# HongMJ1315/Path_Tracing

Hardware: AMD Instinct MI355X
Metric: Msamples/s (paths/s) at 1024^2 x 256spp (higher is better)
Workload: dtype f32; 1 GPU; configs[2]: unidirectional PT + NEE, Cornell-style box + tessellated sphere, 99024 triangles behind a BVH, 1024x1024, 256 spp, depth 4, 1 cone light; parallelism=image tiles 32x32 round-robin over 1 rank(s), RCCL gather to rank 0, seed=1

## Files before the change

### path_tracing_amd/csrc/hpt_host.h

```cpp
#pragma once
#include "../../include/hpt.h"
#include "hpt_scene.h"
#include "pt_kernels.h"
#include "bdpt_kernels.h"
#include "ppm_kernels.h"

#include <hip/hip_runtime.h>
#include <algorithm>
#include <cstring>
#include <string>
#include <vector>

namespace hpt {

int fail(int code, const std::string &msg);

inline int fail_hip(const std::string &what, hipError_t e){
    return fail(e == hipErrorOutOfMemory ? HPT_ERR_NOMEM : HPT_ERR_DEVICE, what + ": " + hipGetErrorString(e));
}

#define HIP_TRY(expr) do { hipError_t e_ = (expr); if(e_ != hipSuccess) return hpt::fail_hip(#expr, e_); } while(0)

template <typename T>
class DevBuf {
// ... 49 lines not shown
        hpt::DevBuf<hpt::DevMaterial> mats; hpt::DevBuf<hpt::DevLight> lights;
        hpt::DevBuf<float4> tri_frames;
        int stack_levels = hpt::kStackDepth;
        std::vector<unsigned char> h_lights, h_spheres, h_tris;
        int nl = 0, ns = 0, nt = 0;
        std::vector<int32_t> g_kind, g_index, g_group;
    } geo;

    struct PassBuffers {
        hpt::DevBuf<float4> org_eta, dir_flags, thr, col; hpt::DevBuf<uint2> rng, hit;
        hpt::DevBuf<float4> org_max, dir, contrib;
        hpt::PathBuf pb{}; hpt::ShadowBuf sb{};
        hpt::DevBuf<uint32_t> queue[2];
        hpt::DevBuf<uint32_t> squeue;
        hpt::DevBuf<uint32_t> lqueue[2];
        hpt::DevBuf<uint32_t> deep_stack;
        hpt::DevBuf<uint32_t> counters;
        uint32_t *h_count = nullptr;
        size_t cap_paths() const { return org_eta.capacity(); }
    };
    struct Workspace {
        PassBuffers pass[hpt::kMaxPipes];
        hipStream_t px_stream[hpt::kMaxPipes] = {}; int px_priority[hpt::kMaxPipes] = {};
        hipEvent_t px_fork = nullptr, px_done[hpt::kMaxPipes] = {};
        const uint32_t *last_counters = nullptr;
        int last_counter_stride = 0;
        int last_budget = 0;
        hpt::DevBuf<float4> accum;
        hpt::DevBuf<hpt::WorkCounters> wc;
        hpt::DevBuf<float> local_own, image_own;
// ... 93 lines not shown
```

### path_tracing_amd/csrc/pt_kernels.h

```cpp
#pragma once
#include <hip/hip_runtime.h>
#include <cstdint>
#include "hpt_scene.h"

namespace hpt {

struct SceneDev {
    const float4 *nodes;
    const uint4 *qnodes;
    const uint4 *wnodes;
    int wide_depth;
    float qorigin[3], qscale[3];
    const float4 *tris;
    const float4 *tri_frames;
    const DevRound *rounds;
    const DevMaterial *mats;
    const DevLight *lights;
    int num_rounds, num_spheres, num_lights, num_tris, num_mats, num_nodes;
};

struct PathBuf {
    float4 *org_eta;
    float4 *dir_flags;
    float4 *thr;
// ... 43 lines not shown
constexpr int kTraceBudget = HPT_TRACE_BUDGET;
constexpr int kTopLevels = HPT_TOP_LEVELS;
constexpr int kTopNodes = 1 << kTopLevels;

void launch_generate(hipStream_t s, const Tiling &tl, const CameraDev &cam, PathBuf pb,
                     uint32_t *qcount, int samples_this_pass, uint32_t first_sample, uint64_t seed,
                     WorkCounters *wc);
void launch_extend(hipStream_t s, const SceneDev &sc, PathBuf pb, const uint32_t *queue, const uint32_t *qcount,
                   uint32_t max_items, int flags, WorkCounters *wc);
void launch_shade(hipStream_t s, const SceneDev &sc, PathBuf pb, const uint32_t *queue, const uint32_t *qcount,
                  uint32_t max_items, uint32_t *next_queue, uint32_t *next_count, ShadowBuf sb, uint32_t *squeue,
                  uint32_t *scount, int max_depth, int max_delta, int roulette, WorkCounters *wc, const PrimaryGen *primary = nullptr,
                  uint32_t max_groups = 0);
void launch_connect(hipStream_t s, const SceneDev &sc, PathBuf pb, ShadowBuf sb, const uint32_t *squeue,
                    const uint32_t *scount, uint32_t max_items, int flags, WorkCounters *wc);
struct TraceSplit { uint32_t *equeue, *ecount, *squeue, *scount; int budget; };
void launch_trace(hipStream_t s, const SceneDev &sc, PathBuf pb, ShadowBuf sb, const uint32_t *equeue,
                  const uint32_t *ecount, uint32_t max_extend, const uint32_t *squeue, const uint32_t *scount,
                  uint32_t max_shadow, int stack_levels, bool count, WorkCounters *wc,
                  const TraceSplit *split = nullptr, const PrimaryGen *primary = nullptr, uint32_t max_groups = 0);
void launch_trace_resume(hipStream_t s, const SceneDev &sc, PathBuf pb, ShadowBuf sb, bool extend, bool shadow,
                         uint32_t max_items, WorkCounters *wc, const TraceSplit &split, const PrimaryGen *primary,
                         uint32_t max_groups, uint32_t *deep_stack);
inline bool resume_walk_fits(const SceneDev &sc){ return 3 * sc.wide_depth + 2 <= kResumeLdsLevels + kDeepLevels; }
size_t resume_deep_stack_words();
void launch_tri_frames(hipStream_t s, const float4 *tris, int num_tris, float4 *frames);
void launch_resolve(hipStream_t s, const Tiling &tl, PathBuf pb, float4 *accum, int samples_this_pass);
void launch_finalize(hipStream_t s, const Tiling &tl, const float4 *accum, float *d_local, float scale);
void launch_untile(hipStream_t s, const Tiling &tl, const float *d_gathered, float *d_image);

void launch_tonemap(hipStream_t s, const float *d_linear, void *d_bytes, unsigned long long num_values, int bgr, const float *d_thresholds);

void launch_probe_functions(hipStream_t s, const float *d_in, int n, float *d_out);
void launch_probe_closest(hipStream_t s, const SceneDev &sc, const float *org, const float *dir, int n, int flags,
                          float *t_out, int32_t *prim_out);
void launch_probe_visibility(hipStream_t s, const SceneDev &sc, const float *p1, const float *p2, int n, int flags,
                             int32_t *vis_out);

// ... 2 lines not shown
```

### path_tracing_amd/csrc/pt_kernels.hip

```cpp
#include "pt_kernels.h"
#include "pt_device_math.h"

namespace hpt {

namespace {

HPT_DEV uint32_t f2u(float f){ return __float_as_uint(f); }
HPT_DEV float u2f(uint32_t u){ return __uint_as_float(u); }
HPT_DEV f3 xyz(float4 v){ return mk3(v.x, v.y, v.z); }

HPT_DEV uint32_t bit_select(uint32_t m, uint32_t a, uint32_t b){ uint32_t r; asm("v_bfi_b32 %0, %1, %2, %3" : "=v"(r) : "v"(m), "v"(a), "v"(b)); return r; }
HPT_DEV float lo16f(uint32_t w){ float r; asm("v_cvt_f32_u32_sdwa %0, %1 dst_sel:DWORD dst_unused:UNUSED_PAD src0_sel:WORD_0" : "=v"(r) : "v"(w)); return r; }
HPT_DEV float hi16f(uint32_t w){ float r; asm("v_cvt_f32_u32_sdwa %0, %1 dst_sel:DWORD dst_unused:UNUSED_PAD src0_sel:WORD_1" : "=v"(r) : "v"(w)); return r; }

HPT_DEV uint32_t lds_push(bool want, uint32_t *lds_counter){
    unsigned long long mask = __ballot(want);
    if(mask == 0ull) return 0u;
    uint32_t lo = (uint32_t) mask, hi = (uint32_t) (mask >> 32);
    uint32_t prefix = __builtin_amdgcn_mbcnt_hi(hi, __builtin_amdgcn_mbcnt_lo(lo, 0u));
    uint32_t base = 0u;
    int leader = __ffsll((long long) mask) - 1;
    if((int) (threadIdx.x & 63u) == leader) base = atomicAdd(lds_counter, (uint32_t) __popcll(mask));
    base = (uint32_t) __shfl((int) base, leader, 64);
    return base + prefix;
// ... 215 lines not shown
        ++rays;
        if(COUNT) tally.wave_steps += wave_max_u32(tally.steps - s0);
    }
    if(COUNT) flush_tally(tally, rays, wc, false);
}

template <bool BRUTE, bool COUNT>
__global__ __launch_bounds__(kBlock)
void k_connect(SceneDev sc, PathBuf pb, ShadowBuf sb, const uint32_t *squeue, const uint32_t *scount, WorkCounters *wc){
    __shared__ uint32_t s_stack[kStackDepth * kBlock];
    uint32_t count = *scount;
    uint32_t *stk = s_stack + threadIdx.x;
    Tally tally; tally.boxes = 0; tally.tris = 0; tally.steps = 0; tally.wave_steps = 0;
    uint32_t rays = 0;
    for(uint32_t i = blockIdx.x * kBlock + threadIdx.x; i < count; i += gridDim.x * kBlock){
        uint32_t path = squeue[i];
        float4 a = sb.org_max[path], b = sb.dir[path];
        uint32_t s0 = tally.steps;
        bool vis = segment_visible<BRUTE, COUNT>(sc, xyz(a), xyz(b), a.w, stk, tally);
        ++rays;
        if(COUNT) tally.wave_steps += wave_max_u32(tally.steps - s0);
        if(vis){
            float4 c = sb.contrib[path];
            float4 col = pb.col[path];
            col.x = col.x + c.x; col.y = col.y + c.y; col.z = col.z + c.z;
            pb.col[path] = col;
        }
    }
    if(COUNT) flush_tally(tally, rays, wc, true);
}

#ifndef HPT_LDS_MATS
#define HPT_LDS_MATS 128
#endif
#ifndef HPT_LDS_LIGHTS
#define HPT_LDS_LIGHTS 32
#endif
#ifndef HPT_SHADE_CHUNK
// ... 13 lines not shown
#ifdef HPT_SHADE_PROFILE
#define HPT_SECTION(set, idx) do { if(wc && HPT_SHADE_PROFILE == (set)){ unsigned long long m_ = __ballot(true); \
    if((int) (threadIdx.x & 63u) == __ffsll((long long) m_) - 1){ atomicAdd(&wc->bd_pairs + 2 * (idx), 1ull); atomicAdd(&wc->bd_pairs + 2 * (idx) + 1, (unsigned long long) __popcll(m_)); } } } while(0)
#else
#define HPT_SECTION(set, idx) do {} while(0)
#endif

template <bool PRIMARY, bool STRIDED>
__global__ __launch_bounds__(kBlock) HPT_SHADE_ATTR
void k_shade(SceneDev sc, PathBuf pb, const uint32_t *queue, const uint32_t *qcount,
             uint32_t *next_queue, uint32_t *next_count, ShadowBuf sb, uint32_t *squeue, uint32_t *scount,
             int max_depth, int max_delta, int roulette, WorkCounters *wc, PrimaryGen pg){
    __shared__ DevMaterial s_mats[kLdsMats];
    __shared__ DevLight s_lights[kLdsLights];
    __shared__ uint32_t s_next[kShadeChunk];
    __shared__ uint32_t s_shadow[kShadeChunk];
    __shared__ uint32_t s_cnt[4];
    __shared__ uint32_t s_stage[kBlock / 64][kNeeWords][64];
    uint32_t (*stage)[64] = s_stage[threadIdx.x >> 6];
    uint32_t staged = 0u;
    const uint32_t lane = threadIdx.x & 63u;
    auto flush_nee = [&](uint32_t n){
        bool want = false; uint32_t spath = 0u;
        if(lane < n){
            HPT_SECTION(2, 3);
            f3 wo_l = mk3(u2f(stage[0][lane]), u2f(stage[1][lane]), u2f(stage[2][lane]));
            f3 wi_l = mk3(u2f(stage[3][lane]), u2f(stage[4][lane]), u2f(stage[5][lane]));
            ShadePre pre; pre.lam_o = u2f(stage[6][lane]);
            const uint32_t mat_i = stage[7][lane], light_i = stage[19][lane];
            f3 thr = mk3(u2f(stage[8][lane]), u2f(stage[9][lane]), u2f(stage[10][lane]));
            const float pdf_light_dir = u2f(stage[11][lane]);
            f3 p1 = mk3(u2f(stage[12][lane]), u2f(stage[13][lane]), u2f(stage[14][lane]));
            f3 p2 = mk3(u2f(stage[15][lane]), u2f(stage[16][lane]), u2f(stage[17][lane]));
            spath = stage[18][lane];
            const DevMaterial dm = (sc.num_mats <= kLdsMats ? s_mats : sc.mats)[mat_i];
            const DevLight &L = (sc.num_lights <= kLdsLights ? s_lights : sc.lights)[light_i & 0x7FFFFFFFu];
            Mat m; m.base = mk3(dm.base[0], dm.base[1], dm.base[2]); m.roughness = dm.roughness; m.metallic = dm.metallic; m.eta = dm.eta;
            pre.diffuse = mk3(dm.diffuse[0], dm.diffuse[1], dm.diffuse[2]);
// ... 4 lines not shown
            f3 contrib;
            if(light_i >> 31) contrib = thr * brdf * illum * mk3(1.0f, 1.0f, 1.0f) * cos_surface * (float) sc.num_lights;
            else {
                float p_l = pdf_light_dir * pdf_light_dir;
                float p_b = pdf_bsdf * pdf_bsdf;
                float mis_w = p_l / fmaxf(p_l + p_b, 1e-8f);
                contrib = thr * brdf * illum * mk3(1.0f, 1.0f, 1.0f) * cos_surface / pdf_light_dir * mis_w;
            }
            if(is_valid_color(contrib)){
                HPT_SECTION(5, 3);
                want = true;
                f3 c = clamp_radiance(contrib, 15.0f);
                f3 diff = p2 - p1;
                float dist = length3(diff);
                f3 dir = diff / dist;
                sb.org_max[spath] = make_float4(p1.x, p1.y, p1.z, dist - 1e-3f);
                sb.dir[spath] = make_float4(dir.x, dir.y, dir.z, 0.0f);
                sb.contrib[spath] = make_float4(c.x, c.y, c.z, 0.0f);
            }
        }
        uint32_t spos = lds_push(want, &s_cnt[1]);
        if(want) s_shadow[spos] = spath;
    };
#ifdef HPT_SHADE_PROFILE
    g_hpt_probe = wc ? &wc->bd_pairs : nullptr;
#endif
    if(threadIdx.x < 4) s_cnt[threadIdx.x] = 0u;
    const bool mats_in_lds = sc.num_mats <= kLdsMats;
    const bool lights_in_lds = sc.num_lights <= kLdsLights;
    if(mats_in_lds){
        const uint32_t *src = (const uint32_t *) sc.mats; uint32_t *dst = (uint32_t *) s_mats;
        for(int w = threadIdx.x; w < sc.num_mats * (int) (sizeof(DevMaterial) / 4); w += kBlock) dst[w] = src[w];
    }
    if(lights_in_lds){
        const uint32_t *src = (const uint32_t *) sc.lights; uint32_t *dst = (uint32_t *) s_lights;
        for(int w = threadIdx.x; w < sc.num_lights * (int) (sizeof(DevLight) / 4); w += kBlock) dst[w] = src[w];
    }
// ... 2 lines not shown
    const DevLight *lights = lights_in_lds ? s_lights : sc.lights;

    uint32_t count = *qcount;
    uint32_t chunk = (count + kShadeTargetGroups - 1) / kShadeTargetGroups;
    chunk = (chunk + kBlock - 1) / kBlock * kBlock;
    chunk = chunk < (uint32_t) kBlock ? (uint32_t) kBlock : (chunk > (uint32_t) kShadeChunk ? (uint32_t) kShadeChunk : chunk);
    uint32_t iters = 0;
    for(uint32_t cb = blockIdx.x; (unsigned long long) cb * chunk < count; cb += gridDim.x){
    if(STRIDED && cb != blockIdx.x){
        __syncthreads();
        if(threadIdx.x < 4) s_cnt[threadIdx.x] = 0u;
        __syncthreads();
    }
    uint32_t begin = cb * chunk;
    uint32_t end = begin + chunk < count ? begin + chunk : count;
    for(uint32_t base = begin; base < end; base += kBlock){
        uint32_t i = base + threadIdx.x;
        bool alive = false, nee = false;
        uint32_t path = 0;
        f3 n_wo = mk3(0, 0, 0), n_wi = mk3(0, 0, 0), n_thr = mk3(0, 0, 0), s_p1 = mk3(0, 0, 0), s_p2 = mk3(0, 0, 0);
        float n_lam = 0.0f, n_pdf_light = 0.0f; uint32_t n_mat = 0u, n_light = 0u;
        if(i < count){
            path = queue ? queue[i] : i;
            ++iters;
            HPT_SECTION(1, 0);
            uint2 h = pb.hit[path];
            uint32_t prim = h.y;
            f3 p_eye = mk3(0, 0, 0), p_dir = mk3(0, 0, 1), first_col = mk3(0, 0, 0); uint64_t p_rs = 0ull;
            if(PRIMARY && !primary_ray(pg, path, p_eye, p_dir, p_rs)) prim = kHitMiss;
            if(prim != kHitMiss){
// ... 200 lines not shown
                }
                staged += k;
            }
        }
        uint32_t qpos = lds_push(alive, &s_cnt[0]);
        if(alive) s_next[qpos] = path;
    }
    if(staged != 0u){ flush_nee(staged); staged = 0u; }
    __syncthreads();
    if(threadIdx.x == 0){
        s_cnt[2] = s_cnt[0] ? atomicAdd(next_count, s_cnt[0]) : 0u;
        s_cnt[3] = s_cnt[1] ? atomicAdd(scount, s_cnt[1]) : 0u;
    }
    __syncthreads();
    for(uint32_t k = threadIdx.x; k < s_cnt[0]; k += kBlock) next_queue[s_cnt[2] + k] = s_next[k];
    for(uint32_t k = threadIdx.x; k < s_cnt[1]; k += kBlock) squeue[s_cnt[3] + k] = s_shadow[k];
    if(!STRIDED) break;
    }
    if(wc){
        unsigned long long v = iters;
        for(int off = 32; off > 0; off >>= 1) v += __shfl_down(v, off, 64);
        if((threadIdx.x & 63u) == 0u && v) atomicAdd(&wc->path_iters, v);
    }
}

__global__ __launch_bounds__(kBlock)
void k_resolve(Tiling tl, PathBuf pb, float4 *accum, int samples){
    uint32_t p = blockIdx.x * kBlock + threadIdx.x;
    if(p >= (uint32_t) tl.n_local) return;
    float4 a = accum[p];
    f3 sum = mk3(a.x, a.y, a.z);
// ... 84 lines not shown
#if HPT_TRACE_WAVES > 0
#define HPT_TRACE_ATTR __attribute__((amdgpu_waves_per_eu(HPT_TRACE_WAVES, 8)))
#else
#define HPT_TRACE_ATTR
#endif
constexpr int kTraceChunk = 2048;
constexpr uint32_t kDoneCode = 0xFFFFFFFEu;
constexpr int kRefillMin = 56;
constexpr int kNodeMin = 4;
constexpr uint32_t kTraceShortQueue = 1u << 20;

template <bool ANY, bool COUNT, bool RESUME, bool TOP, bool PRIMARY>
HPT_DEV void trace_chunk(const SceneDev &sc, PathBuf pb, ShadowBuf sb, const uint32_t *queue,
                         uint32_t end, uint32_t *stk, uint32_t *s_next, int refill_min, int node_min, WorkCounters *wc,
                         uint32_t budget, uint32_t *s_long, uint32_t *s_nlong, const uint4 *top, const PrimaryGen &pg,
                         uint32_t *deep, uint32_t deep_stride){
    bool active = false, exhausted = false;
    uint32_t path = 0u, cur = 0u, steps = 0u;
    int sp = 0;
    f3 ro = mk3(0, 0, 0), rd = mk3(0, 0, 1);
    float ix = 0, iy = 0, iz = 0, ox = 0, oy = 0, oz = 0;
    uint32_t mx = 0u, my = 0u, mz = 0u;
    float tmax = 0.0f, limit = 0.0f, best_t = 1e20f;
    uint32_t best_prim = kHitMiss, best_ord = 0xFFFFFFFFu;
    unsigned long long n_lane_steps = 0, n_wave_steps = 0, n_boxes = 0, n_tris = 0, n_rays = 0, n_leaf_lane = 0, n_leaf_wave = 0;
    const uint32_t lane = threadIdx.x & 63u;
    const uint32_t step_limit = budget != 0u ? budget : 0xFFFFFFFFu;
    for(;;){
        if(!RESUME && budget != 0u){
            bool defer = active && steps >= budget;
            unsigned long long dm = __ballot(defer);
            if(dm != 0ull){
                uint32_t dn = (uint32_t) __popcll(dm);
                uint32_t dprefix = __builtin_amdgcn_mbcnt_hi((uint32_t) (dm >> 32), __builtin_amdgcn_mbcnt_lo((uint32_t) dm, 0u));
                int dleader = __ffsll((long long) dm) - 1;
                uint32_t dbase = 0u;
                if((int) lane == dleader) dbase = atomicAdd(s_nlong, dn);
                dbase = (uint32_t) __shfl((int) dbase, dleader, 64);
                if(defer){
                    s_long[dbase + dprefix] = path;
                    if(!ANY) pb.hit[path] = make_uint2(f2u(best_t), best_prim);
                    active = false;
                }
            }
        }
        unsigned long long idle = __ballot(!active);
        if(idle != 0ull && !exhausted && (idle == ~0ull || __popcll(idle) >= refill_min)){
            uint32_t n = (uint32_t) __popcll(idle);
            uint32_t prefix = __builtin_amdgcn_mbcnt_hi((uint32_t) (idle >> 32), __builtin_amdgcn_mbcnt_lo((uint32_t) idle, 0u));
            int leader = __ffsll((long long) idle) - 1;
            uint32_t base = 0u;
            if((int) lane == leader) base = atomicAdd(s_next, n);
            base = (uint32_t) __shfl((int) base, leader, 64);
            exhausted = base + n >= end;
            if(!active){
                uint32_t i = base + prefix;
                if(i < end){
                    path = queue ? queue[i] : i;
                    bool start = true;
                    if(ANY){
                        float4 a = sb.org_max[path], b = sb.dir[path];
                        ro = xyz(a); rd = xyz(b); tmax = a.w;
                        if(COUNT && !RESUME) n_rays += 1;
                        for(int r = 0; r < (RESUME ? 0 : sc.num_spheres); ++r){
                            DevRound rr = sc.rounds[r];
                            float t;
                            if(hit_sphere(ro, rd, mk3(rr.c[0], rr.c[1], rr.c[2]), rr.r, tmax, t) && t > 1e-3f && (rr.flags & 1u)) start = false;
                        }
                        limit = tmax;
                    } else {
                        bool outside;
                        if(PRIMARY){
                            uint64_t rs_unused;
                            outside = !primary_ray(pg, path, ro, rd, rs_unused);
                            if(outside && !RESUME) pb.hit[path] = make_uint2(f2u(1e20f), kHitMiss);
                        } else {
                            float4 o = pb.org_eta[path], d = pb.dir_flags[path];
                            ro = xyz(o); rd = xyz(d);
                            outside = (f2u(d.w) & 2u) != 0u;
                        }
                        if(outside) start = false;
                        else if(RESUME){
                            uint2 h = pb.hit[path];
                            best_t = u2f(h.x); best_prim = h.y; best_ord = 0xFFFFFFFFu;
                            if(best_prim != kHitMiss)
                                best_ord = (best_prim & kHitRoundFlag) ? (best_prim & ~kHitRoundFlag) : f2u(sc.tris[(size_t) best_prim * 3].w);
                            limit = best_t;
                        } else {
                            if(COUNT) n_rays += 1;
                            best_t = 1e20f; best_prim = kHitMiss; best_ord = 0xFFFFFFFFu;
                            for(int r = 0; r < sc.num_rounds; ++r){
                                DevRound rr = sc.rounds[r];
                                float t;
                                if(hit_sphere(ro, rd, mk3(rr.c[0], rr.c[1], rr.c[2]), rr.r, 1e20f, t) && t < best_t){
                                    best_t = t; best_prim = kHitRoundFlag | (uint32_t) r; best_ord = (uint32_t) r;
                                }
                            }
                            limit = best_t;
                        }
                    }
                    if(start){
                        float dx = fabsf(rd.x) > 1e-20f ? rd.x : copysignf(1e-20f, rd.x);
                        float dy = fabsf(rd.y) > 1e-20f ? rd.y : copysignf(1e-20f, rd.y);
// ... 115 lines not shown
                            }
                        }
                    }
                }
                if(ANY && blocked) finished = true;
                else if(sp > 0){
                    --sp;
                    cur = (RESUME && sp >= kResumeLdsLevels) ? deep[(size_t) (sp - kResumeLdsLevels) * deep_stride] : stk[sp * kBlock];
                }
                else finished = true;
            }
            if(finished){
                active = false;
                if(!ANY) pb.hit[path] = make_uint2(f2u(best_t), best_prim);
                else if(!blocked){
                    float4 c = sb.contrib[path];
                    float4 col = pb.col[path];
                    col.x = col.x + c.x; col.y = col.y + c.y; col.z = col.z + c.z;
                    pb.col[path] = col;
                }
            }
        }
    }
    if(COUNT){
        for(int off = 32; off > 0; off >>= 1){
            n_boxes += __shfl_down(n_boxes, off, 64); n_tris += __shfl_down(n_tris, off, 64);
            n_rays += __shfl_down(n_rays, off, 64); n_lane_steps += __shfl_down(n_lane_steps, off, 64);
            n_wave_steps += __shfl_down(n_wave_steps, off, 64); n_leaf_lane += __shfl_down(n_leaf_lane, off, 64);
            n_leaf_wave += __shfl_down(n_leaf_wave, off, 64);
        }
        if(lane == 0u){
            if(n_boxes) atomicAdd(ANY ? &wc->boxes_shadow : &wc->boxes_closest, n_boxes);
            if(n_tris) atomicAdd(ANY ? &wc->tris_shadow : &wc->tris_closest, n_tris);
            if(n_rays) atomicAdd(ANY ? &wc->shadow_rays : &wc->closest_rays, n_rays);
            if(n_lane_steps) atomicAdd(ANY ? &wc->lane_steps_shadow : &wc->lane_steps_closest, n_lane_steps);
            if(n_wave_steps) atomicAdd(ANY ? &wc->wave_steps_shadow : &wc->wave_steps_closest, n_wave_steps);
            if(n_leaf_lane) atomicAdd(ANY ? &wc->leaf_lane_shadow : &wc->leaf_lane_closest, n_leaf_lane);
            if(n_leaf_wave) atomicAdd(ANY ? &wc->leaf_wave_shadow : &wc->leaf_wave_closest, n_leaf_wave);
        }
    }
}

struct LongQueues { uint32_t *equeue, *ecount, *squeue, *scount; uint32_t budget; };

template <bool COUNT, bool RESUME, bool TOP, bool PRIMARY>
__global__ __launch_bounds__(kBlock) HPT_TRACE_ATTR
void k_trace(SceneDev sc, PathBuf pb, ShadowBuf sb, const uint32_t *equeue, const uint32_t *ecount_ptr,
             const uint32_t *squeue, const uint32_t *scount_ptr, uint32_t chunk_rays, int refill_min, int node_min,
             int stack_words, LongQueues lq, WorkCounters *wc, PrimaryGen pg, uint32_t *deep){
    extern __shared__ uint32_t s_dyn_stack[];
    __shared__ uint32_t s_next, s_nlong, s_gbase;
    __shared__ uint4 s_top[TOP ? kTopNodes * 2 : 1];
    uint32_t *s_long = s_dyn_stack + stack_words;
    if(TOP){
        const uint32_t words = (uint32_t) (sc.num_nodes < kTopNodes ? sc.num_nodes : kTopNodes) * 2u;
        for(uint32_t i = threadIdx.x; i < words; i += kBlock) s_top[i] = sc.qnodes[i];
    }
    uint32_t ecount = ecount_ptr ? *ecount_ptr : 0u, scount = scount_ptr ? *scount_ptr : 0u;
    uint32_t ce = ecount >= kTraceShortQueue ? chunk_rays : (uint32_t) kBlock;
    uint32_t cs = scount >= kTraceShortQueue ? chunk_rays : (uint32_t) kBlock;
    uint32_t ne = (ecount + ce - 1) / ce, ns = (scount + cs - 1) / cs;
    for(uint32_t bid = blockIdx.x; bid < ne + ns; bid += gridDim.x){
        bool shadow = bid >= ne;
        uint32_t chunk = shadow ? bid - ne : bid;
        uint32_t csize = shadow ? cs : ce;
        uint32_t begin = chunk * csize;
        uint32_t total = shadow ? scount : ecount;
        uint32_t end = begin + csize < total ? begin + csize : total;
        if(threadIdx.x == 0){ s_next = begin; s_nlong = 0u; }
        __syncthreads();
        uint32_t *deep_lane = RESUME ? deep + (size_t) blockIdx.x * kBlock + threadIdx.x : nullptr;
        const uint32_t deep_stride = gridDim.x * kBlock;
        if(shadow) trace_chunk<true, COUNT, RESUME, TOP, false>(sc, pb, sb, squeue, end, s_dyn_stack + threadIdx.x, &s_next, refill_min, node_min, wc,
                                                                lq.budget, s_long, &s_nlong, s_top, pg, deep_lane, deep_stride);
        else trace_chunk<false, COUNT, RESUME, TOP, PRIMARY>(sc, pb, sb, equeue, end, s_dyn_stack + threadIdx.x, &s_next, refill_min, node_min, wc,
                                                             lq.budget, s_long, &s_nlong, s_top, pg, deep_lane, deep_stride);
        __syncthreads();
        if(!RESUME && lq.budget != 0u){
            uint32_t n = s_nlong;
            if(n != 0u){
                if(threadIdx.x == 0) s_gbase = atomicAdd(shadow ? lq.scount : lq.ecount, n);
                __syncthreads();
                uint32_t *dst = (shadow ? lq.squeue : lq.equeue) + s_gbase;
                for(uint32_t i = threadIdx.x; i < n; i += kBlock) dst[i] = s_long[i];
            }
        }
        __syncthreads();
    }
}

template <bool BRUTE>
__global__ __launch_bounds__(kBlock)
void k_probe_closest(SceneDev sc, const float *org, const float *dir, int n, float *t_out, int32_t *prim_out){
    __shared__ uint32_t s_stack[kStackDepth * kBlock];
    int i = blockIdx.x * kBlock + threadIdx.x;
    if(i >= n) return;
    Tally tally; tally.boxes = 0; tally.tris = 0; tally.steps = 0; tally.wave_steps = 0;
    float t; uint32_t prim;
    closest_hit<BRUTE, false>(sc, mk3(org[3 * i], org[3 * i + 1], org[3 * i + 2]), mk3(dir[3 * i], dir[3 * i + 1], dir[3 * i + 2]),
// ... 121 lines not shown
    auto groups = [&](uint32_t items){
        uint32_t a = (items + chunk - 1) / chunk;
        uint32_t shortest = items < kTraceShortQueue ? items : kTraceShortQueue;
        uint32_t b = (shortest + kBlock - 1) / kBlock;
        return a > b ? a : b;
    };
    uint32_t g = (ecount ? groups(max_extend) : 0u) + (scount ? groups(max_shadow) : 0u);
    if(g == 0u) return;
    if(max_groups != 0u && g > max_groups) g = max_groups;
    if(stack_levels < 1) stack_levels = 1;
    if(stack_levels > kStackDepth) stack_levels = kStackDepth;
    int stack_words = (stack_levels + 1) * kBlock;
    LongQueues lq{};
    if(split && split->budget > 0 && !count){
        lq.equeue = split->equeue; lq.ecount = split->ecount; lq.squeue = split->squeue; lq.scount = split->scount;
        lq.budget = (uint32_t) split->budget;
        if(stack_levels > split->budget) stack_words = (split->budget + 1) * kBlock;
    }
    size_t lds = (size_t) stack_words * sizeof(uint32_t) + (lq.budget ? (size_t) chunk * sizeof(uint32_t) : 0);
    const bool top = lq.budget != 0u && lq.budget <= (uint32_t) kTopLevels;
    PrimaryGen none{};
    const PrimaryGen &pg = primary ? *primary : none;
#define HPT_LAUNCH_TRACE(C, T, P) hipLaunchKernelGGL((k_trace<C, false, T, P>), dim3(g), dim3(kBlock), lds, s, sc, pb, sb, equeue, ecount, squeue, \
                                                     scount, chunk, kRefillMin, kNodeMin, stack_words, lq, wc, pg, (uint32_t *) nullptr)
    if(count) HPT_LAUNCH_TRACE(true, false, false);
    else if(top && primary) HPT_LAUNCH_TRACE(false, true, true);
    else if(top) HPT_LAUNCH_TRACE(false, true, false);
    else if(primary) HPT_LAUNCH_TRACE(false, false, true);
    else HPT_LAUNCH_TRACE(false, false, false);
#undef HPT_LAUNCH_TRACE
}

void launch_trace_resume(hipStream_t s, const SceneDev &sc, PathBuf pb, ShadowBuf sb, bool extend, bool shadow,
                         uint32_t max_items, WorkCounters *wc, const TraceSplit &split, const PrimaryGen *primary,
                         uint32_t max_groups, uint32_t *deep_stack){
    if(!extend && !shadow) return;
    const int stack_words = (kResumeLdsLevels + 1) * kBlock;
    const size_t lds = (size_t) stack_words * sizeof(uint32_t);
    uint32_t per = (max_items + kBlock - 1) / kBlock;
    uint64_t g = (uint64_t) per * ((extend ? 1u : 0u) + (shadow ? 1u : 0u));
    uint32_t g2 = g < kResumeMaxGroups ? (uint32_t) (g < 1u ? 1u : g) : kResumeMaxGroups;
    if(max_groups != 0u && g2 > max_groups) g2 = max_groups;
    LongQueues none{};
    PrimaryGen no_primary{};
    const uint32_t *eq = extend ? split.equeue : nullptr, *ec = extend ? split.ecount : nullptr;
    const uint32_t *sq = shadow ? split.squeue : nullptr, *scn = shadow ? split.scount : nullptr;
#define HPT_LAUNCH_RESUME(P, PG) hipLaunchKernelGGL((k_trace<false, true, false, P>), dim3(g2), dim3(kBlock), lds, s, sc, pb, sb, eq, ec, sq, scn, \
                                                    kLongChunk, kWideRefillMin, kWideNodeMin, stack_words, none, wc, PG, deep_stack)
    if(primary && extend) HPT_LAUNCH_RESUME(true, *primary);
    else HPT_LAUNCH_RESUME(false, no_primary);
#undef HPT_LAUNCH_RESUME
}

size_t resume_deep_stack_words(){ return (size_t) kDeepLevels * kResumeMaxGroups * kBlock; }

void launch_tri_frames(hipStream_t s, const float4 *tris, int num_tris, float4 *frames){
    if(num_tris <= 0) return;
    hipLaunchKernelGGL(k_tri_frames, dim3((num_tris + kBlock - 1) / kBlock), dim3(kBlock), 0, s, tris, num_tris, frames);
}

void launch_resolve(hipStream_t s, const Tiling &tl, PathBuf pb, float4 *accum, int samples_this_pass){
    uint32_t g = ((uint32_t) tl.n_local + kBlock - 1) / kBlock;
    hipLaunchKernelGGL(k_resolve, dim3(g), dim3(kBlock), 0, s, tl, pb, accum, samples_this_pass);
}

void launch_finalize(hipStream_t s, const Tiling &tl, const float4 *accum, float *d_local, float divisor){
// ... 37 lines not shown
```

### path_tracing_amd/csrc/render_ppm.cpp

```cpp
#include "hpt_host.h"

#include <new>

using namespace hpt;

namespace {

void ppm_scene_bounds(hpt_scene *s){
    if(s->pm.bounds_ready) return;
    float mn[3] = { 1e9f, 1e9f, 1e9f }, mx[3] = { -1e9f, -1e9f, -1e9f };
    for(int i = 0; i < s->geo.ns; ++i){
        float c[4]; memcpy(c, s->geo.h_spheres.data() + (size_t) i * HPT_SPHERE_BYTES, 16);
        for(int a = 0; a < 3; ++a){ mx[a] = std::max(mx[a], c[a] + c[3]); mn[a] = std::min(mn[a], c[a] - c[3]); }
    }
    for(int i = 0; i < s->geo.nt; ++i){
        float v[9]; memcpy(v, s->geo.h_tris.data() + (size_t) i * HPT_TRIANGLE_BYTES, 36);
        for(int a = 0; a < 3; ++a){
            mx[a] = std::max({ mx[a], v[a], v[3 + a], v[6 + a] });
            mn[a] = std::min({ mn[a], v[a], v[3 + a], v[6 + a] });
        }
    }
    for(int a = 0; a < 3; ++a){ s->pm.min[a] = mn[a]; s->pm.max[a] = mx[a]; }
    s->pm.bounds_ready = true;
}
// ... 57 lines not shown
}

void ppm_mark(hpt_scene *s, const PpmRun &r, int pass, int k){ if(r.timek) hipEventRecord(s->pm.marks[(size_t) pass * 5 + k], nullptr); }

int ppm_phases(hpt_scene *s, const PpmRun &r, int pass, uint32_t pidx){
    const hpt_params &P = r.P;
    const PpmFrame &fr = r.fr;
    const uint32_t n_local = r.n_local, n_ph = r.n_ph, n_dep = r.n_dep;
    const int M = r.M, light_depth = r.light_depth;
    hipStream_t st = nullptr;
    PassBuffers &w = s->ws.pass[0];
    uint32_t *eq = w.counters.get(), *elc = w.counters.get() + M, *pq = w.counters.get() + 2 * M, *plc = w.counters.get() + 3 * M;
    uint32_t *hp_count = r.hp_count(s), *no_shadow = w.counters.get() + 4 * M + 1;
    const int budget = resume_walk_fits(s->geo.sd) ? kTraceBudget : 0;
    auto trace = [&](int it, const uint32_t *queue, uint32_t *cnt, uint32_t *lcnt, uint32_t max_items){
        TraceSplit split{ w.lqueue[0].get(), &lcnt[it], w.lqueue[1].get(), no_shadow, budget };
        launch_trace(st, s->geo.sd, w.pb, w.sb, queue, &cnt[it], max_items, nullptr, nullptr, 0, s->geo.stack_levels, false, nullptr, &split, nullptr, 0u);
        if(budget > 0) launch_trace_resume(st, s->geo.sd, w.pb, w.sb, true, false, max_items, nullptr, split, nullptr, 0u, w.deep_stack.get());
    };
    auto queue_empty = [&](const uint32_t *cnt, bool &empty) -> int {
        HIP_TRY(hipMemcpyAsync(w.h_count, cnt, sizeof(uint32_t), hipMemcpyDeviceToHost, st));
        HIP_TRY(hipStreamSynchronize(st));
        empty = *w.h_count == 0u;
        return HPT_OK;
    };
    HIP_TRY(hipMemsetAsync(w.counters.get(), 0, (size_t) r.n_counters * sizeof(uint32_t), st));
    ppm_mark(s, r, pass, 0);
    launch_generate(st, r.tl, r.cam, w.pb, &eq[0], 1, pidx, P.seed ^ kPpmEyeKey, nullptr);
    int cur = 0;
    for(int it = 0; it < r.eye_iters; ++it){
        if(it >= 1){ bool empty; if(int rc = queue_empty(&eq[it], empty)) return rc; if(empty) break; }
        const uint32_t *q = it == 0 ? nullptr : w.queue[cur].get();
        trace(it, q, eq, elc, n_local);
// ... 242 lines not shown
```

### path_tracing_amd/csrc/render_pt.cpp

```cpp
#include "hpt_host.h"

using namespace hpt;

namespace {

constexpr double kBytesPerPathSlot = 148.0;

int ensure_pass(PassBuffers &w, size_t paths, int n_counters){
    const hipError_t e = reserve_all(paths, w.org_eta, w.dir_flags, w.thr, w.col, w.rng, w.hit, w.org_max, w.dir, w.contrib,
                                     w.queue[0], w.queue[1], w.squeue, w.lqueue[0], w.lqueue[1]);
    w.pb = PathBuf{ w.org_eta.get(), w.dir_flags.get(), w.thr.get(), w.col.get(), w.rng.get(), w.hit.get() };
    w.sb = ShadowBuf{ w.org_max.get(), w.dir.get(), w.contrib.get() };
    if(e != hipSuccess) return fail_hip("path workspace", e);
    HIP_TRY(w.deep_stack.reserve(resume_deep_stack_words()));
    HIP_TRY(w.counters.reserve((size_t) n_counters));
    if(!w.h_count) HIP_TRY(hipHostMalloc((void **) &w.h_count, 64));
    return HPT_OK;
}

int ensure_pipes(hpt_scene::Workspace &ws, hipStream_t caller, int npipes){
    int pr_least = 0, pr_greatest = 0, pr_caller = 0;
    HIP_TRY(hipDeviceGetStreamPriorityRange(&pr_least, &pr_greatest));
    if(hipStreamGetPriority(caller, &pr_caller) != hipSuccess){ (void) hipGetLastError(); pr_caller = 0; }
    std::vector<int> levels;
    for(int l = pr_greatest; l <= pr_least; ++l) if(l != pr_caller) levels.push_back(l);
    if(levels.empty()) levels.push_back(pr_caller);
    for(int k = 1; k < npipes; ++k){
// ... 80 lines not shown

    WorkCounters *wc = count ? s->ws.wc.get() : nullptr;
    reset_render_stats(s);

    int budget = (P.reserved >> 1) & 0x3F;
    budget = budget == 0 ? kTraceBudget : (budget == 0x3F ? 0 : budget);
    if(count || brute || !resume_walk_fits(s->geo.sd)) budget = 0;
    s->ws.last_budget = budget;
    const int roulette = (flags & HPT_FLAG_RUSSIAN_ROULETTE) ? 1 : 0;

    HIP_TRY(hipMemsetAsync(s->ws.wc.get(), 0, sizeof(WorkCounters), stream));
    HIP_TRY(hipMemsetAsync(s->ws.accum.get(), 0, (size_t) tl.n_local * sizeof(float4), stream));
    HIP_TRY(hipEventRecord(s->tm.ev_start, stream));

    struct Pass {
        PathBuf pb; ShadowBuf sb; uint32_t *queue[2], *squeue, *lqueue[2], *deep_stack; uint32_t *counters, *h_count; hipStream_t st;
        int sthis = 0, cur = 0, pending_shadow = -1; uint32_t slots = 0; PrimaryGen primary{};
        uint32_t *qcnt = nullptr, *scnt = nullptr, *lecnt = nullptr, *lscnt = nullptr;
    };
    Pass pipe[kMaxPipes]{};
    for(int k = 0; k < npipes; ++k){
        const PassBuffers &w = s->ws.pass[k];
        Pass &q = pipe[k];
        q.pb = w.pb; q.sb = w.sb; q.queue[0] = w.queue[0].get(); q.queue[1] = w.queue[1].get(); q.squeue = w.squeue.get();
        q.lqueue[0] = w.lqueue[0].get(); q.lqueue[1] = w.lqueue[1].get();
        q.deep_stack = w.deep_stack.get();
        q.counters = w.counters.get(); q.h_count = w.h_count; q.st = k == 0 ? stream : s->ws.px_stream[k];
    }
    for(Pass &q : pipe){
        if(!q.counters) continue;
        q.qcnt = q.counters;
        q.scnt = q.counters + (max_iters + 2);
        q.lecnt = q.counters + 2 * (max_iters + 2);
        q.lscnt = q.counters + 3 * (max_iters + 2);
    }

    const bool in_flight_primaries = !count && !brute;
    auto begin_pass = [&](Pass &q, int done) -> int {
        q.sthis = std::min(spass, spp - done);
// ... 6 lines not shown
        } else {
            LaunchTimer t(s, q.st, timek, 3);
            launch_generate(q.st, tl, cam, q.pb, &q.qcnt[0], q.sthis, q.primary.first_sample, P.seed, wc);
        }
        return HPT_OK;
    };
    const uint32_t blind_groups = (flags & HPT_FLAG_NO_HOST_WAIT) ? (uint32_t) std::max(s->num_cus, 1) * 8u : 0u;
    auto iteration = [&](Pass &q, int it){
        const uint32_t *eq = it == 0 ? nullptr : q.queue[q.cur];
        const PrimaryGen *primary = (it == 0 && in_flight_primaries) ? &q.primary : nullptr;
        const uint32_t cap = it >= eye_depth ? blind_groups : 0u;
        if(brute){
            LaunchTimer t(s, q.st, timek, 0);
            launch_extend(q.st, s->geo.sd, q.pb, eq, &q.qcnt[it], q.slots, kflags, wc);
        } else {
            TraceSplit split{ q.lqueue[0], &q.lecnt[it], q.lqueue[1], &q.lscnt[it], budget };
            { LaunchTimer t(s, q.st, timek, 0);
              launch_trace(q.st, s->geo.sd, q.pb, q.sb, eq, &q.qcnt[it], q.slots, q.squeue,
                           q.pending_shadow >= 0 ? &q.scnt[q.pending_shadow] : nullptr, q.slots, s->geo.stack_levels, count, wc, &split, primary, cap); }
            if(split.budget > 0){
                LaunchTimer t(s, q.st, timek, 4);
                launch_trace_resume(q.st, s->geo.sd, q.pb, q.sb, true, q.pending_shadow >= 0, q.slots, wc, split, primary, cap, q.deep_stack);
            }
            q.pending_shadow = -1;
        }
        { LaunchTimer t(s, q.st, timek, 1);
          launch_shade(q.st, s->geo.sd, q.pb, eq, &q.qcnt[it], q.slots, q.queue[q.cur ^ 1],
                       &q.qcnt[it + 1], q.sb, q.squeue, &q.scnt[it], eye_depth, P.max_delta, roulette, wc, primary, cap); }
        if(brute){
            LaunchTimer t(s, q.st, timek, 2);
            launch_connect(q.st, s->geo.sd, q.pb, q.sb, q.squeue, &q.scnt[it], q.slots, kflags, wc);
        } else q.pending_shadow = it;
        q.cur ^= 1;
    };
    const bool no_host_wait = (flags & HPT_FLAG_NO_HOST_WAIT) != 0;
    auto tails = [&](int npipes) -> int {
        bool live[kMaxPipes]; int nlive = npipes;
// ... 2 lines not shown
            const bool look = !no_host_wait && ((it - eye_depth) & 1) == 0;
            if(look) for(int k = 0; k < npipes; ++k) if(live[k])
                HIP_TRY(hipMemcpyAsync(pipe[k].h_count, &pipe[k].qcnt[it], sizeof(uint32_t), hipMemcpyDeviceToHost, pipe[k].st));
            for(int k = 0; k < npipes; ++k){
                if(!live[k]) continue;
                if(look){
                    HIP_TRY(hipStreamSynchronize(pipe[k].st));
                    if(*pipe[k].h_count == 0u){ live[k] = false; --nlive; continue; }
                }
                iteration(pipe[k], it);
            }
        }
        for(int k = 0; k < npipes; ++k){
            Pass &q = pipe[k];
            if(q.pending_shadow < 0) continue;
            TraceSplit split{ q.lqueue[0], &q.lecnt[max_iters], q.lqueue[1], &q.lscnt[max_iters], budget };
            { LaunchTimer t(s, q.st, timek, 2);
              launch_trace(q.st, s->geo.sd, q.pb, q.sb, nullptr, nullptr, 0, q.squeue, &q.scnt[q.pending_shadow], q.slots,
                           s->geo.stack_levels, count, wc, &split, nullptr, blind_groups); }
            if(split.budget > 0){
                LaunchTimer t(s, q.st, timek, 4);
                launch_trace_resume(q.st, s->geo.sd, q.pb, q.sb, false, true, q.slots, wc, split, nullptr, blind_groups, q.deep_stack);
            }
        }
        return HPT_OK;
    };

    for(int done = 0; done < spp; done += spass * npipes){
        int active = 0;
        while(active < npipes && done + active * spass < spp) ++active;
        if(active > 1){
            HIP_TRY(hipEventRecord(s->ws.px_fork, stream));
            for(int k = 1; k < active; ++k) HIP_TRY(hipStreamWaitEvent(s->ws.px_stream[k], s->ws.px_fork, 0));
        }
        for(int k = 0; k < active; ++k){ rc = begin_pass(pipe[k], done + k * spass); if(rc) return rc; }
        for(int it = 0; it < eye_depth && it < max_iters; ++it)
            for(int k = 0; k < active; ++k) iteration(pipe[k], it);
// ... 38 lines not shown
```

Before: 2159 Msamples/s.

## Store deferred long rays and shadow records compactly, indexed by chunk position

Deferred extension rays now write their origin, direction, current best hit and ordinal into dedicated long-ray record buffers. The resume kernel reads these records directly instead of regenerating primary rays or re-reading path state and the triangle ordinal. Shadow-ray records are written at chunk-local positions with the path slot packed into contrib.w, so the shade kernel no longer needs an LDS indirection list and shadow tracing reads contiguous memory. This costs more device memory per path slot and extra record writes when rays are deferred.

```diff
diff --git a/path_tracing_amd/csrc/hpt_host.h b/path_tracing_amd/csrc/hpt_host.h
--- a/path_tracing_amd/csrc/hpt_host.h
+++ b/path_tracing_amd/csrc/hpt_host.h
@@ -87,6 +87,8 @@
         hpt::DevBuf<uint32_t> queue[2];
         hpt::DevBuf<uint32_t> squeue;
         hpt::DevBuf<uint32_t> lqueue[2];
+        hpt::DevBuf<float4> long_org, long_dir; hpt::DevBuf<uint2> long_ids;
+        hpt::LongRayBuf lr{};
         hpt::DevBuf<uint32_t> deep_stack;
         hpt::DevBuf<uint32_t> counters;
         uint32_t *h_count = nullptr;
diff --git a/path_tracing_amd/csrc/pt_kernels.h b/path_tracing_amd/csrc/pt_kernels.h
--- a/path_tracing_amd/csrc/pt_kernels.h
+++ b/path_tracing_amd/csrc/pt_kernels.h
@@ -81,14 +81,18 @@
                   uint32_t max_groups = 0);
 void launch_connect(hipStream_t s, const SceneDev &sc, PathBuf pb, ShadowBuf sb, const uint32_t *squeue,
                     const uint32_t *scount, uint32_t max_items, int flags, WorkCounters *wc);
-struct TraceSplit { uint32_t *equeue, *ecount, *squeue, *scount; int budget; };
+struct LongRayBuf {
+    float4 *org_t;
+    float4 *dir_prim;
+    uint2 *slot_ord;
+};
+struct TraceSplit { uint32_t *equeue, *ecount, *squeue, *scount; int budget; LongRayBuf rec; };
 void launch_trace(hipStream_t s, const SceneDev &sc, PathBuf pb, ShadowBuf sb, const uint32_t *equeue,
                   const uint32_t *ecount, uint32_t max_extend, const uint32_t *squeue, const uint32_t *scount,
                   uint32_t max_shadow, int stack_levels, bool count, WorkCounters *wc,
                   const TraceSplit *split = nullptr, const PrimaryGen *primary = nullptr, uint32_t max_groups = 0);
 void launch_trace_resume(hipStream_t s, const SceneDev &sc, PathBuf pb, ShadowBuf sb, bool extend, bool shadow,
-                         uint32_t max_items, WorkCounters *wc, const TraceSplit &split, const PrimaryGen *primary,
-                         uint32_t max_groups, uint32_t *deep_stack);
+                         uint32_t max_items, WorkCounters *wc, const TraceSplit &split, uint32_t max_groups, uint32_t *deep_stack);
 inline bool resume_walk_fits(const SceneDev &sc){ return 3 * sc.wide_depth + 2 <= kResumeLdsLevels + kDeepLevels; }
 size_t resume_deep_stack_words();
 void launch_tri_frames(hipStream_t s, const float4 *tris, int num_tris, float4 *frames);
diff --git a/path_tracing_amd/csrc/pt_kernels.hip b/path_tracing_amd/csrc/pt_kernels.hip
--- a/path_tracing_amd/csrc/pt_kernels.hip
+++ b/path_tracing_amd/csrc/pt_kernels.hip
@@ -253,14 +253,15 @@
     Tally tally; tally.boxes = 0; tally.tris = 0; tally.steps = 0; tally.wave_steps = 0;
     uint32_t rays = 0;
     for(uint32_t i = blockIdx.x * kBlock + threadIdx.x; i < count; i += gridDim.x * kBlock){
-        uint32_t path = squeue[i];
-        float4 a = sb.org_max[path], b = sb.dir[path];
+        uint32_t rec = squeue[i];
+        float4 a = sb.org_max[rec], b = sb.dir[rec];
         uint32_t s0 = tally.steps;
         bool vis = segment_visible<BRUTE, COUNT>(sc, xyz(a), xyz(b), a.w, stk, tally);
         ++rays;
         if(COUNT) tally.wave_steps += wave_max_u32(tally.steps - s0);
         if(vis){
-            float4 c = sb.contrib[path];
+            float4 c = sb.contrib[rec];
+            uint32_t path = f2u(c.w);
             float4 col = pb.col[path];
             col.x = col.x + c.x; col.y = col.y + c.y; col.z = col.z + c.z;
             pb.col[path] = col;
@@ -304,14 +305,15 @@
     __shared__ DevMaterial s_mats[kLdsMats];
     __shared__ DevLight s_lights[kLdsLights];
     __shared__ uint32_t s_next[kShadeChunk];
-    __shared__ uint32_t s_shadow[kShadeChunk];
     __shared__ uint32_t s_cnt[4];
     __shared__ uint32_t s_stage[kBlock / 64][kNeeWords][64];
     uint32_t (*stage)[64] = s_stage[threadIdx.x >> 6];
     uint32_t staged = 0u;
     const uint32_t lane = threadIdx.x & 63u;
+    uint32_t rec_base = 0u;
     auto flush_nee = [&](uint32_t n){
         bool want = false; uint32_t spath = 0u;
+        f3 s_o = mk3(0, 0, 0), s_d = mk3(0, 0, 0), s_c = mk3(0, 0, 0); float s_max = 0.0f;
         if(lane < n){
             HPT_SECTION(2, 3);
             f3 wo_l = mk3(u2f(stage[0][lane]), u2f(stage[1][lane]), u2f(stage[2][lane]));
@@ -346,13 +348,16 @@
                 f3 diff = p2 - p1;
                 float dist = length3(diff);
                 f3 dir = diff / dist;
-                sb.org_max[spath] = make_float4(p1.x, p1.y, p1.z, dist - 1e-3f);
-                sb.dir[spath] = make_float4(dir.x, dir.y, dir.z, 0.0f);
-                sb.contrib[spath] = make_float4(c.x, c.y, c.z, 0.0f);
+                s_o = p1; s_d = dir; s_c = c; s_max = dist - 1e-3f;
             }
         }
         uint32_t spos = lds_push(want, &s_cnt[1]);
-        if(want) s_shadow[spos] = spath;
+        if(want){
+            const uint32_t rec = rec_base + spos;
+            sb.org_max[rec] = make_float4(s_o.x, s_o.y, s_o.z, s_max);
+            sb.dir[rec] = make_float4(s_d.x, s_d.y, s_d.z, 0.0f);
+            sb.contrib[rec] = make_float4(s_c.x, s_c.y, s_c.z, u2f(spath));
+        }
     };
 #ifdef HPT_SHADE_PROFILE
     g_hpt_probe = wc ? &wc->bd_pairs : nullptr;
@@ -385,6 +390,7 @@
     }
     uint32_t begin = cb * chunk;
     uint32_t end = begin + chunk < count ? begin + chunk : count;
+    rec_base = begin;
     for(uint32_t base = begin; base < end; base += kBlock){
         uint32_t i = base + threadIdx.x;
         bool alive = false, nee = false;
@@ -615,7 +621,7 @@
     }
     __syncthreads();
     for(uint32_t k = threadIdx.x; k < s_cnt[0]; k += kBlock) next_queue[s_cnt[2] + k] = s_next[k];
-    for(uint32_t k = threadIdx.x; k < s_cnt[1]; k += kBlock) squeue[s_cnt[3] + k] = s_shadow[k];
+    for(uint32_t k = threadIdx.x; k < s_cnt[1]; k += kBlock) squeue[s_cnt[3] + k] = begin + k;
     if(!STRIDED) break;
     }
     if(wc){
@@ -730,9 +736,10 @@
 HPT_DEV void trace_chunk(const SceneDev &sc, PathBuf pb, ShadowBuf sb, const uint32_t *queue,
                          uint32_t end, uint32_t *stk, uint32_t *s_next, int refill_min, int node_min, WorkCounters *wc,
                          uint32_t budget, uint32_t *s_long, uint32_t *s_nlong, const uint4 *top, const PrimaryGen &pg,
-                         uint32_t *deep, uint32_t deep_stride){
+                         uint32_t *deep, uint32_t deep_stride, LongRayBuf lr, uint32_t rec_base){
     bool active = false, exhausted = false;
     uint32_t path = 0u, cur = 0u, steps = 0u;
+    uint32_t rec = 0u;
     int sp = 0;
     f3 ro = mk3(0, 0, 0), rd = mk3(0, 0, 1);
     float ix = 0, iy = 0, iz = 0, ox = 0, oy = 0, oz = 0;
@@ -754,8 +761,13 @@
                 if((int) lane == dleader) dbase = atomicAdd(s_nlong, dn);
                 dbase = (uint32_t) __shfl((int) dbase, dleader, 64);
                 if(defer){
-                    s_long[dbase + dprefix] = path;
-                    if(!ANY) pb.hit[path] = make_uint2(f2u(best_t), best_prim);
+                    if(ANY) s_long[dbase + dprefix] = rec;
+                    else {
+                        const uint32_t lrec = rec_base + dbase + dprefix;
+                        lr.org_t[lrec] = make_float4(ro.x, ro.y, ro.z, best_t);
+                        lr.dir_prim[lrec] = make_float4(rd.x, rd.y, rd.z, u2f(best_prim));
+                        lr.slot_ord[lrec] = make_uint2(path, best_ord);
+                    }
                     active = false;
                 }
             }
@@ -772,10 +784,17 @@
             if(!active){
                 uint32_t i = base + prefix;
                 if(i < end){
-                    path = queue ? queue[i] : i;
+                    const uint32_t entry = queue ? queue[i] : i;
                     bool start = true;
-                    if(ANY){
-                        float4 a = sb.org_max[path], b = sb.dir[path];
+                    if(!ANY && RESUME){
+                        const float4 a = lr.org_t[entry], b = lr.dir_prim[entry];
+                        const uint2 c = lr.slot_ord[entry];
+                        ro = xyz(a); rd = xyz(b);
+                        best_t = a.w; best_prim = f2u(b.w); best_ord = c.y; path = c.x;
+                        limit = best_t;
+                    } else if(ANY){
+                        rec = entry;
+                        float4 a = sb.org_max[rec], b = sb.dir[rec];
                         ro = xyz(a); rd = xyz(b); tmax = a.w;
                         if(COUNT && !RESUME) n_rays += 1;
                         for(int r = 0; r < (RESUME ? 0 : sc.num_spheres); ++r){
@@ -785,24 +804,19 @@
                         }
                         limit = tmax;
                     } else {
+                        path = entry;
                         bool outside;
                         if(PRIMARY){
                             uint64_t rs_unused;
                             outside = !primary_ray(pg, path, ro, rd, rs_unused);
-                            if(outside && !RESUME) pb.hit[path] = make_uint2(f2u(1e20f), kHitMiss);
+                            if(outside) pb.hit[path] = make_uint2(f2u(1e20f), kHitMiss);
                         } else {
                             float4 o = pb.org_eta[path], d = pb.dir_flags[path];
                             ro = xyz(o); rd = xyz(d);
                             outside = (f2u(d.w) & 2u) != 0u;
                         }
                         if(outside) start = false;
-                        else if(RESUME){
-                            uint2 h = pb.hit[path];
-                            best_t = u2f(h.x); best_prim = h.y; best_ord = 0xFFFFFFFFu;
-                            if(best_prim != kHitMiss)
-                                best_ord = (best_prim & kHitRoundFlag) ? (best_prim & ~kHitRoundFlag) : f2u(sc.tris[(size_t) best_prim * 3].w);
-                            limit = best_t;
-                        } else {
+                        else {
                             if(COUNT) n_rays += 1;
                             best_t = 1e20f; best_prim = kHitMiss; best_ord = 0xFFFFFFFFu;
                             for(int r = 0; r < sc.num_rounds; ++r){
@@ -948,10 +962,11 @@
                 active = false;
                 if(!ANY) pb.hit[path] = make_uint2(f2u(best_t), best_prim);
                 else if(!blocked){
-                    float4 c = sb.contrib[path];
-                    float4 col = pb.col[path];
+                    float4 c = sb.contrib[rec];
+                    const uint32_t slot = f2u(c.w);
+                    float4 col = pb.col[slot];
                     col.x = col.x + c.x; col.y = col.y + c.y; col.z = col.z + c.z;
-                    pb.col[path] = col;
+                    pb.col[slot] = col;
                 }
             }
         }
@@ -975,7 +990,7 @@
     }
 }
 
-struct LongQueues { uint32_t *equeue, *ecount, *squeue, *scount; uint32_t budget; };
+struct LongQueues { uint32_t *equeue, *ecount, *squeue, *scount; uint32_t budget; LongRayBuf rec; };
 
 template <bool COUNT, bool RESUME, bool TOP, bool PRIMARY>
 __global__ __launch_bounds__(kBlock) HPT_TRACE_ATTR
@@ -1006,9 +1021,9 @@
         uint32_t *deep_lane = RESUME ? deep + (size_t) blockIdx.x * kBlock + threadIdx.x : nullptr;
         const uint32_t deep_stride = gridDim.x * kBlock;
         if(shadow) trace_chunk<true, COUNT, RESUME, TOP, false>(sc, pb, sb, squeue, end, s_dyn_stack + threadIdx.x, &s_next, refill_min, node_min, wc,
-                                                                lq.budget, s_long, &s_nlong, s_top, pg, deep_lane, deep_stride);
+                                                                lq.budget, s_long, &s_nlong, s_top, pg, deep_lane, deep_stride, lq.rec, begin);
         else trace_chunk<false, COUNT, RESUME, TOP, PRIMARY>(sc, pb, sb, equeue, end, s_dyn_stack + threadIdx.x, &s_next, refill_min, node_min, wc,
-                                                             lq.budget, s_long, &s_nlong, s_top, pg, deep_lane, deep_stride);
+                                                             lq.budget, s_long, &s_nlong, s_top, pg, deep_lane, deep_stride, lq.rec, begin);
         __syncthreads();
         if(!RESUME && lq.budget != 0u){
             uint32_t n = s_nlong;
@@ -1016,7 +1031,7 @@
                 if(threadIdx.x == 0) s_gbase = atomicAdd(shadow ? lq.scount : lq.ecount, n);
                 __syncthreads();
                 uint32_t *dst = (shadow ? lq.squeue : lq.equeue) + s_gbase;
-                for(uint32_t i = threadIdx.x; i < n; i += kBlock) dst[i] = s_long[i];
+                for(uint32_t i = threadIdx.x; i < n; i += kBlock) dst[i] = shadow ? s_long[i] : begin + i;
             }
         }
         __syncthreads();
@@ -1168,7 +1183,7 @@
     LongQueues lq{};
     if(split && split->budget > 0 && !count){
         lq.equeue = split->equeue; lq.ecount = split->ecount; lq.squeue = split->squeue; lq.scount = split->scount;
-        lq.budget = (uint32_t) split->budget;
+        lq.budget = (uint32_t) split->budget; lq.rec = split->rec;
         if(stack_levels > split->budget) stack_words = (split->budget + 1) * kBlock;
     }
     size_t lds = (size_t) stack_words * sizeof(uint32_t) + (lq.budget ? (size_t) chunk * sizeof(uint32_t) : 0);
@@ -1186,8 +1201,7 @@
 }
 
 void launch_trace_resume(hipStream_t s, const SceneDev &sc, PathBuf pb, ShadowBuf sb, bool extend, bool shadow,
-                         uint32_t max_items, WorkCounters *wc, const TraceSplit &split, const PrimaryGen *primary,
-                         uint32_t max_groups, uint32_t *deep_stack){
+                         uint32_t max_items, WorkCounters *wc, const TraceSplit &split, uint32_t max_groups, uint32_t *deep_stack){
     if(!extend && !shadow) return;
     const int stack_words = (kResumeLdsLevels + 1) * kBlock;
     const size_t lds = (size_t) stack_words * sizeof(uint32_t);
@@ -1195,15 +1209,13 @@
     uint64_t g = (uint64_t) per * ((extend ? 1u : 0u) + (shadow ? 1u : 0u));
     uint32_t g2 = g < kResumeMaxGroups ? (uint32_t) (g < 1u ? 1u : g) : kResumeMaxGroups;
     if(max_groups != 0u && g2 > max_groups) g2 = max_groups;
-    LongQueues none{};
+    LongQueues records{};
+    records.rec = split.rec;
     PrimaryGen no_primary{};
     const uint32_t *eq = extend ? split.equeue : nullptr, *ec = extend ? split.ecount : nullptr;
     const uint32_t *sq = shadow ? split.squeue : nullptr, *scn = shadow ? split.scount : nullptr;
-#define HPT_LAUNCH_RESUME(P, PG) hipLaunchKernelGGL((k_trace<false, true, false, P>), dim3(g2), dim3(kBlock), lds, s, sc, pb, sb, eq, ec, sq, scn, \
-                                                    kLongChunk, kWideRefillMin, kWideNodeMin, stack_words, none, wc, PG, deep_stack)
-    if(primary && extend) HPT_LAUNCH_RESUME(true, *primary);
-    else HPT_LAUNCH_RESUME(false, no_primary);
-#undef HPT_LAUNCH_RESUME
+    hipLaunchKernelGGL((k_trace<false, true, false, false>), dim3(g2), dim3(kBlock), lds, s, sc, pb, sb, eq, ec, sq, scn,
+                       kLongChunk, kWideRefillMin, kWideNodeMin, stack_words, records, wc, no_primary, deep_stack);
 }
 
 size_t resume_deep_stack_words(){ return (size_t) kDeepLevels * kResumeMaxGroups * kBlock; }
diff --git a/path_tracing_amd/csrc/render_ppm.cpp b/path_tracing_amd/csrc/render_ppm.cpp
--- a/path_tracing_amd/csrc/render_ppm.cpp
+++ b/path_tracing_amd/csrc/render_ppm.cpp
@@ -95,9 +95,9 @@
     uint32_t *hp_count = r.hp_count(s), *no_shadow = w.counters.get() + 4 * M + 1;
     const int budget = resume_walk_fits(s->geo.sd) ? kTraceBudget : 0;
     auto trace = [&](int it, const uint32_t *queue, uint32_t *cnt, uint32_t *lcnt, uint32_t max_items){
-        TraceSplit split{ w.lqueue[0].get(), &lcnt[it], w.lqueue[1].get(), no_shadow, budget };
+        TraceSplit split{ w.lqueue[0].get(), &lcnt[it], w.lqueue[1].get(), no_shadow, budget, w.lr };
         launch_trace(st, s->geo.sd, w.pb, w.sb, queue, &cnt[it], max_items, nullptr, nullptr, 0, s->geo.stack_levels, false, nullptr, &split, nullptr, 0u);
-        if(budget > 0) launch_trace_resume(st, s->geo.sd, w.pb, w.sb, true, false, max_items, nullptr, split, nullptr, 0u, w.deep_stack.get());
+        if(budget > 0) launch_trace_resume(st, s->geo.sd, w.pb, w.sb, true, false, max_items, nullptr, split, 0u, w.deep_stack.get());
     };
     auto queue_empty = [&](const uint32_t *cnt, bool &empty) -> int {
         HIP_TRY(hipMemcpyAsync(w.h_count, cnt, sizeof(uint32_t), hipMemcpyDeviceToHost, st));
diff --git a/path_tracing_amd/csrc/render_pt.cpp b/path_tracing_amd/csrc/render_pt.cpp
--- a/path_tracing_amd/csrc/render_pt.cpp
+++ b/path_tracing_amd/csrc/render_pt.cpp
@@ -4,13 +4,14 @@
 
 namespace {
 
-constexpr double kBytesPerPathSlot = 148.0;
+constexpr double kBytesPerPathSlot = 188.0;
 
 int ensure_pass(PassBuffers &w, size_t paths, int n_counters){
     const hipError_t e = reserve_all(paths, w.org_eta, w.dir_flags, w.thr, w.col, w.rng, w.hit, w.org_max, w.dir, w.contrib,
-                                     w.queue[0], w.queue[1], w.squeue, w.lqueue[0], w.lqueue[1]);
+                                     w.queue[0], w.queue[1], w.squeue, w.lqueue[0], w.lqueue[1], w.long_org, w.long_dir, w.long_ids);
     w.pb = PathBuf{ w.org_eta.get(), w.dir_flags.get(), w.thr.get(), w.col.get(), w.rng.get(), w.hit.get() };
     w.sb = ShadowBuf{ w.org_max.get(), w.dir.get(), w.contrib.get() };
+    w.lr = LongRayBuf{ w.long_org.get(), w.long_dir.get(), w.long_ids.get() };
     if(e != hipSuccess) return fail_hip("path workspace", e);
     HIP_TRY(w.deep_stack.reserve(resume_deep_stack_words()));
     HIP_TRY(w.counters.reserve((size_t) n_counters));
@@ -121,7 +122,7 @@
     HIP_TRY(hipEventRecord(s->tm.ev_start, stream));
 
     struct Pass {
-        PathBuf pb; ShadowBuf sb; uint32_t *queue[2], *squeue, *lqueue[2], *deep_stack; uint32_t *counters, *h_count; hipStream_t st;
+        PathBuf pb; ShadowBuf sb; LongRayBuf lr; uint32_t *queue[2], *squeue, *lqueue[2], *deep_stack; uint32_t *counters, *h_count; hipStream_t st;
         int sthis = 0, cur = 0, pending_shadow = -1; uint32_t slots = 0; PrimaryGen primary{};
         uint32_t *qcnt = nullptr, *scnt = nullptr, *lecnt = nullptr, *lscnt = nullptr;
     };
@@ -129,7 +130,7 @@
     for(int k = 0; k < npipes; ++k){
         const PassBuffers &w = s->ws.pass[k];
         Pass &q = pipe[k];
-        q.pb = w.pb; q.sb = w.sb; q.queue[0] = w.queue[0].get(); q.queue[1] = w.queue[1].get(); q.squeue = w.squeue.get();
+        q.pb = w.pb; q.sb = w.sb; q.lr = w.lr; q.queue[0] = w.queue[0].get(); q.queue[1] = w.queue[1].get(); q.squeue = w.squeue.get();
         q.lqueue[0] = w.lqueue[0].get(); q.lqueue[1] = w.lqueue[1].get();
         q.deep_stack = w.deep_stack.get();
         q.counters = w.counters.get(); q.h_count = w.h_count; q.st = k == 0 ? stream : s->ws.px_stream[k];
@@ -166,13 +167,13 @@
             LaunchTimer t(s, q.st, timek, 0);
             launch_extend(q.st, s->geo.sd, q.pb, eq, &q.qcnt[it], q.slots, kflags, wc);
         } else {
-            TraceSplit split{ q.lqueue[0], &q.lecnt[it], q.lqueue[1], &q.lscnt[it], budget };
+            TraceSplit split{ q.lqueue[0], &q.lecnt[it], q.lqueue[1], &q.lscnt[it], budget, q.lr };
             { LaunchTimer t(s, q.st, timek, 0);
               launch_trace(q.st, s->geo.sd, q.pb, q.sb, eq, &q.qcnt[it], q.slots, q.squeue,
                            q.pending_shadow >= 0 ? &q.scnt[q.pending_shadow] : nullptr, q.slots, s->geo.stack_levels, count, wc, &split, primary, cap); }
             if(split.budget > 0){
                 LaunchTimer t(s, q.st, timek, 4);
-                launch_trace_resume(q.st, s->geo.sd, q.pb, q.sb, true, q.pending_shadow >= 0, q.slots, wc, split, primary, cap, q.deep_stack);
+                launch_trace_resume(q.st, s->geo.sd, q.pb, q.sb, true, q.pending_shadow >= 0, q.slots, wc, split, cap, q.deep_stack);
             }
             q.pending_shadow = -1;
         }
@@ -205,13 +206,13 @@
         for(int k = 0; k < npipes; ++k){
             Pass &q = pipe[k];
             if(q.pending_shadow < 0) continue;
-            TraceSplit split{ q.lqueue[0], &q.lecnt[max_iters], q.lqueue[1], &q.lscnt[max_iters], budget };
+            TraceSplit split{ q.lqueue[0], &q.lecnt[max_iters], q.lqueue[1], &q.lscnt[max_iters], budget, q.lr };
             { LaunchTimer t(s, q.st, timek, 2);
               launch_trace(q.st, s->geo.sd, q.pb, q.sb, nullptr, nullptr, 0, q.squeue, &q.scnt[q.pending_shadow], q.slots,
                            s->geo.stack_levels, count, wc, &split, nullptr, blind_groups); }
             if(split.budget > 0){
                 LaunchTimer t(s, q.st, timek, 4);
-                launch_trace_resume(q.st, s->geo.sd, q.pb, q.sb, false, true, q.slots, wc, split, nullptr, blind_groups, q.deep_stack);
+                launch_trace_resume(q.st, s->geo.sd, q.pb, q.sb, false, true, q.slots, wc, split, blind_groups, q.deep_stack);
             }
         }
         return HPT_OK;
```

Result: faster. 2444 Msamples/s, median of 6 (+13.2%).
